# GenjiB/AVSiam

Measured on AMD Instinct MI355X. Metric: AV pretrain samples/sec (ViT-B/16, 75% mask), higher is better.
Workload: dtype bf16; 1 GPU; AVSiam pretrain step (contrastive + MAE passes, 2x Adam), ViT-B/16, 10 frames x196 + 512 audio tokens, 75% mask, batch 64/GPU; global_batch=64, frames=10, parallelism=dp1, residual_gradient_stream=bf16

## Files before the change

### avsiam_amd/csrc/gemm.hip

```cpp
#include "common.h"
#include <stdlib.h>
#include <type_traits>
#include <algorithm>
#include <numeric>

#define GLOBAL_AS __attribute__((address_space(1)))
#define LDS_AS __attribute__((address_space(3)))

constexpr int BM = 128, BN = 128, BK = 64;

struct GemmNtArgs {
    const bf16_t* A; long long lda;
    const bf16_t* B; long long ldb;
    int M, N, K;
    const float* bias;
    const float* res; long long ldr; const int* res_idx;
    const bf16_t* aux; long long ldaux;
    void* out; long long ldo; int out_f32;
    bf16_t* out2; long long ldo2;
    float alpha; int act;
    int scale_cols; float col_scale;
    float* colsum;
    int m_full;
    int m_split; const bf16_t* B2; const float* bias2; float* colsum2;
    uint8_t* out8; long long ldo8; float out8_scale;
    const float* qa; const float* qw; const float* qw2; float* q8;
    float q8_seen;
    int tb;
    int aux8;
};
#define GP8_BIAS 0.1296875f
#define GP8_STEPS 202.0f


typedef __attribute__((ext_vector_type(4))) uint32_t u32x4;

#ifndef NT8_ABLATE
#define NT8_ABLATE 0
#endif
#if NT8_ABLATE == 1
#define NT_STORE(ptr, val) asm volatile("" ::"v"(val))
#else
#define NT_STORE(ptr, val) *(ptr) = (val)
#endif

__device__ __forceinline__ void epi_apply4(float alpha, int ACT, float (&v)[4], const float4& bias4, uint2 p,
                                           bool has_res, f32x4 r) {
    v[0] += bias4.x; v[1] += bias4.y; v[2] += bias4.z; v[3] += bias4.w;
    if (ACT == 2) {
        v[0] *= __uint_as_float(p.x << 16);
        v[1] *= __uint_as_float(p.x & 0xffff0000u);
        v[2] *= __uint_as_float(p.y << 16);
        v[3] *= __uint_as_float(p.y & 0xffff0000u);
    }
    if (has_res) { v[0] += r[0]; v[1] += r[1]; v[2] += r[2]; v[3] += r[3]; }
    v[0] *= alpha; v[1] *= alpha; v[2] *= alpha; v[3] *= alpha;
}

template <int OFF>
__device__ __forceinline__ void epi_lds_w128(unsigned addr, const f32x4& v) {
    asm volatile("ds_write_b128 %0, %1 offset:%2" ::"v"(addr), "v"(v), "n"(OFF) : "memory");
}
template <int OFF>
__device__ __forceinline__ void epi_lds_r128(f32x4& v, unsigned addr) {
    asm volatile("ds_read_b128 %0, %1 offset:%2" : "=&v"(v) : "v"(addr), "n"(OFF) : "memory");
}
__device__ __forceinline__ void epi_lds_wait() {
    asm volatile("s_waitcnt lgkmcnt(0)" ::: "memory");
    __builtin_amdgcn_sched_barrier(0);
}

template <int MI>
struct EpiPrefetch {
    static constexpr int RG = 1;
    static constexpr int AG = MI < 4 ? MI : 4;
    static constexpr int NB = 3;
    f32x4 rs[NB][RG][4];
    u32x4 ax[AG][2];
};

template <int MI>
__device__ __forceinline__ void epi_load_res(const GemmNtArgs& a, f32x4 (&rs)[EpiPrefetch<MI>::RG][4], int grp, int lane, int mw0, int nw0) {
    const int n = nw0 + (lane & 15) * 4, rq = lane >> 4;
    if (a.res_idx) {
        int rrow[EpiPrefetch<MI>::RG][4];
#pragma unroll
        for (int mj = 0; mj < EpiPrefetch<MI>::RG; ++mj)
#pragma unroll
            for (int i = 0; i < 4; ++i) rrow[mj][i] = a.res_idx[min(mw0 + (grp * EpiPrefetch<MI>::RG + mj) * 16 + i * 4 + rq, a.M - 1)];
#pragma unroll
        for (int mj = 0; mj < EpiPrefetch<MI>::RG; ++mj)
#pragma unroll
            for (int i = 0; i < 4; ++i) rs[mj][i] = *reinterpret_cast<const f32x4*>(a.res + (long long)rrow[mj][i] * a.ldr + n);
    } else {
#pragma unroll
        for (int mj = 0; mj < EpiPrefetch<MI>::RG; ++mj)
#pragma unroll
            for (int i = 0; i < 4; ++i) {
                const int m = min(mw0 + (grp * EpiPrefetch<MI>::RG + mj) * 16 + i * 4 + rq, a.M - 1);
                rs[mj][i] = *reinterpret_cast<const f32x4*>(a.res + (long long)m * a.ldr + n);
            }
    }
}

template <int MI>
__device__ __forceinline__ void epi_load_aux(const GemmNtArgs& a, u32x4 (&ax)[EpiPrefetch<MI>::AG][2], int grp, int lane, int mw0, int nw0) {
    const int n = nw0 + (lane & 7) * 8, rq = lane >> 3;
#pragma unroll
    for (int mj = 0; mj < EpiPrefetch<MI>::AG; ++mj)
#pragma unroll
        for (int i = 0; i < 2; ++i) {
            const int m = min(mw0 + (grp * EpiPrefetch<MI>::AG + mj) * 16 + i * 8 + rq, a.M - 1);
            if (a.aux8) {
                const uint2 c = *reinterpret_cast<const uint2*>(reinterpret_cast<const uint8_t*>(a.aux) + (size_t)m * a.ldaux + n);
                ax[mj][i] = u32x4{c.x, c.y, 0u, 0u};
            } else
            ax[mj][i] = *reinterpret_cast<const u32x4*>(a.aux + (size_t)m * a.ldaux + n);
        }
}

template <int ACT, int MI>
__device__ __forceinline__ void nt_epilogue_prefetch(const GemmNtArgs& a, EpiPrefetch<MI>& pf, int lane, int mw0, int nw0) {
    if (ACT == 0 && a.out_f32 && a.res) {
#pragma unroll
        for (int g = 0; g < EpiPrefetch<MI>::NB - 1 && g < MI / EpiPrefetch<MI>::RG; ++g) epi_load_res<MI>(a, pf.rs[g], g, lane, mw0, nw0);
    }
}

__device__ __forceinline__ void nt_epilogue_stage_bias(const GemmNtArgs& a, char* smem, int wave, int lane, int mw0, int nw0) {
    float* sbias = reinterpret_cast<float*>(smem) + (blockDim.x >> 6) * (16 * 68) + wave * 64;
    const float* bias = mw0 >= a.m_split ? a.bias2 : a.bias;
    sbias[lane] = bias ? bias[nw0 + lane] : 0.f;
}

template <int ACT, int MI, int Q8 = 0>
__device__ __forceinline__ void nt_epilogue(const GemmNtArgs& a, f32x4 (&acc)[4][MI], EpiPrefetch<MI>& pf, char* smem, int wave, int lane,
                                            int mw0, int nw0, const int nrow = MI * 16) {
    const int fr = lane & 15, fq = lane >> 4;
    const unsigned smem_lds = (unsigned)(size_t)(LDS_AS const char*)smem;
    const unsigned stg_lds = smem_lds + wave * (16 * 68) * 4;
    const unsigned sbias_lds = smem_lds + ((blockDim.x >> 6) * (16 * 68) + wave * 64) * 4;
    const unsigned waddr = stg_lds + (fr * 68 + fq * 4) * 4;
    const float alpha = nw0 < a.scale_cols ? a.alpha * a.col_scale : a.alpha;
    float* const colsum = mw0 >= a.m_split ? a.colsum2 : a.colsum;
    if (ACT == 0 && a.out_f32) {
        const int cc = (lane & 15) * 4, rq = lane >> 4;
        const int n = nw0 + cc;
        float* stg = reinterpret_cast<float*>(smem) + wave * (16 * 68);
        const float* sbias = reinterpret_cast<const float*>(smem) + (blockDim.x >> 6) * (16 * 68) + wave * 64;
        constexpr int RG = EpiPrefetch<MI>::RG, NG = MI / RG, NB = EpiPrefetch<MI>::NB;
#pragma unroll
        for (int g = 0; g < NG; ++g) {
            if (g * RG * 16 >= nrow) continue;
            if (a.res && g + NB - 1 < NG) epi_load_res<MI>(a, pf.rs[(g + NB - 1) % NB], g + NB - 1, lane, mw0, nw0);
#pragma unroll
            for (int mj = 0; mj < RG; ++mj) {
                const int mi = g * RG + mj;
#pragma unroll
                for (int ni = 0; ni < 4; ++ni) *reinterpret_cast<f32x4*>(stg + fr * 68 + ni * 16 + fq * 4) = acc[ni][mi];
#pragma unroll
                for (int i = 0; i < 4; ++i) {
                    const int rr = i * 4 + rq;
                    const float4 t = *reinterpret_cast<const float4*>(stg + rr * 68 + cc);
                    const int m = mw0 + mi * 16 + rr;
                    if (m >= a.M) continue;
                    float v[4] = {t.x, t.y, t.z, t.w};
                    const float4 bias4 = *reinterpret_cast<const float4*>(sbias + cc);
                    epi_apply4(alpha, 0, v, bias4, make_uint2(0, 0), a.res != nullptr, pf.rs[g % NB][mj][i]);
                    NT_STORE(reinterpret_cast<f32x4*>(reinterpret_cast<float*>(a.out) + (size_t)m * a.ldo + n), (f32x4{v[0], v[1], v[2], v[3]}));
                }
            }
        }
    } else {
        const int cc = (lane & 7) * 8, rq = lane >> 3;
        const int n = nw0 + cc;
        const unsigned raddr = stg_lds + (rq * 68 + cc) * 4, baddr = sbias_lds + cc * 4;
        constexpr int AG = EpiPrefetch<MI>::AG, NG = MI / AG;
        float cs[8] = {0.f, 0.f, 0.f, 0.f, 0.f, 0.f, 0.f, 0.f};
        const float q8s = (Q8 != 0 && a.out8) ? a.out8_scale : 0.f;
        const float q8seen = a.q8_seen;
        float q8max = 0.f;
#pragma unroll
        for (int g = 0; g < NG; ++g) {
            if (g * AG * 16 >= nrow) continue;
            if (ACT == 2) epi_load_aux<MI>(a, pf.ax, g, lane, mw0, nw0);
#pragma unroll
            for (int mj = 0; mj < AG; ++mj) {
                const int mi = g * AG + mj;
                if (mi * 16 >= nrow) continue;
                epi_lds_w128<0>(waddr, acc[0][mi]); epi_lds_w128<64>(waddr, acc[1][mi]);
                epi_lds_w128<128>(waddr, acc[2][mi]); epi_lds_w128<192>(waddr, acc[3][mi]);
                f32x4 tq[2][2], bq[2];
                epi_lds_r128<0>(tq[0][0], raddr); epi_lds_r128<16>(tq[0][1], raddr);
                epi_lds_r128<2176>(tq[1][0], raddr); epi_lds_r128<2176 + 16>(tq[1][1], raddr);
                epi_lds_r128<0>(bq[0], baddr); epi_lds_r128<16>(bq[1], baddr);
                epi_lds_wait();
#pragma unroll
                for (int i = 0; i < 2; ++i) {
                    const int rr = i * 8 + rq;
                    const int m = mw0 + mi * 16 + rr;
                    if (m >= a.M) continue;
                    float v0[4] = {tq[i][0][0], tq[i][0][1], tq[i][0][2], tq[i][0][3]}, v1[4] = {tq[i][1][0], tq[i][1][1], tq[i][1][2], tq[i][1][3]};
                    u32x4 ax = {0, 0, 0, 0};
                    if (ACT == 2) ax = pf.ax[mj][i];
                    const f32x4 r0 = {0.f, 0.f, 0.f, 0.f}, r1 = r0;
                    const float4 bias_lo = make_float4(bq[0][0], bq[0][1], bq[0][2], bq[0][3]), bias_hi = make_float4(bq[1][0], bq[1][1], bq[1][2], bq[1][3]);
                    if (ACT == 2 && Q8 != 1 && a.aux8) {
                        auto dec = [](float b) { return fmaf(b, 1.0f / GP8_STEPS, -GP8_BIAS); };
                        const float g0[4] = {dec((float)((ax[0] >> 0) & 0xffu)), dec((float)((ax[0] >> 8) & 0xffu)),
                                             dec((float)((ax[0] >> 16) & 0xffu)), dec((float)((ax[0] >> 24) & 0xffu))};
                        const float g1[4] = {dec((float)((ax[1] >> 0) & 0xffu)), dec((float)((ax[1] >> 8) & 0xffu)),
                                             dec((float)((ax[1] >> 16) & 0xffu)), dec((float)((ax[1] >> 24) & 0xffu))};
                        epi_apply4(alpha, 0, v0, bias_lo, make_uint2(0, 0), false, r0);
                        epi_apply4(alpha, 0, v1, bias_hi, make_uint2(0, 0), false, r1);
#pragma unroll
                        for (int j = 0; j < 4; ++j) { v0[j] *= g0[j]; v1[j] *= g1[j]; }
                    } else {
                    epi_apply4(alpha, ACT, v0, bias_lo, make_uint2(ax[0], ax[1]), false, r0);
                    epi_apply4(alpha, ACT, v1, bias_hi, make_uint2(ax[2], ax[3]), false, r1);
                    }
                    if (colsum) {
#pragma unroll
                        for (int j = 0; j < 4; ++j) { cs[j] += v0[j]; cs[4 + j] += v1[j]; }
                    }
                    uint4 o;
                    if (ACT == 1) {
                        o.x = pack_bf2(gelu_erf_grad(v0[0]), gelu_erf_grad(v0[1])); o.y = pack_bf2(gelu_erf_grad(v0[2]), gelu_erf_grad(v0[3]));
                        o.z = pack_bf2(gelu_erf_grad(v1[0]), gelu_erf_grad(v1[1])); o.w = pack_bf2(gelu_erf_grad(v1[2]), gelu_erf_grad(v1[3]));
                    } else {
                        o.x = pack_bf2(v0[0], v0[1]); o.y = pack_bf2(v0[2], v0[3]);
                        o.z = pack_bf2(v1[0], v1[1]); o.w = pack_bf2(v1[2], v1[3]);
                    }
                    if (ACT == 1 && Q8 != 2 && a.aux8) {
                        auto enc = [](float g, unsigned sel, unsigned old) { return __builtin_amdgcn_cvt_pk_u8_f32(fmaf(g, GP8_STEPS, GP8_BIAS * GP8_STEPS), sel, old); };
                        unsigned c0 = enc(gelu_erf_grad(v0[0]), 0, 0); c0 = enc(gelu_erf_grad(v0[1]), 1, c0); c0 = enc(gelu_erf_grad(v0[2]), 2, c0); c0 = enc(gelu_erf_grad(v0[3]), 3, c0);
                        unsigned c1 = enc(gelu_erf_grad(v1[0]), 0, 0); c1 = enc(gelu_erf_grad(v1[1]), 1, c1); c1 = enc(gelu_erf_grad(v1[2]), 2, c1); c1 = enc(gelu_erf_grad(v1[3]), 3, c1);
                        *reinterpret_cast<uint2*>(reinterpret_cast<uint8_t*>(a.out) + (size_t)m * a.ldo + n) = make_uint2(c0, c1);
                    } else
                    if (Q8 != 2 || a.out) NT_STORE(reinterpret_cast<u32x4*>(reinterpret_cast<bf16_t*>(a.out) + (size_t)m * a.ldo + n), (u32x4{o.x, o.y, o.z, o.w}));
                    if (Q8 == 2 && ACT != 1 && a.out8) {
                        auto c8 = [&](float x) { q8max = fmaxf(q8max, fabsf(x)); return __builtin_amdgcn_fmed3f(x * q8s, -57344.f, 57344.f); };
                        int w0 = __builtin_amdgcn_cvt_pk_bf8_f32(c8(v0[0]), c8(v0[1]), 0, false);
                        w0 = __builtin_amdgcn_cvt_pk_bf8_f32(c8(v0[2]), c8(v0[3]), w0, true);
                        int w1 = __builtin_amdgcn_cvt_pk_bf8_f32(c8(v1[0]), c8(v1[1]), 0, false);
                        w1 = __builtin_amdgcn_cvt_pk_bf8_f32(c8(v1[2]), c8(v1[3]), w1, true);
                        *reinterpret_cast<uint2*>(a.out8 + (size_t)m * a.ldo8 + n) = make_uint2((unsigned)w0, (unsigned)w1);
                    }
                    if (ACT == 1) {
                        uint4 gq;
                        gq.x = pack_bf2(gelu_erf(v0[0]), gelu_erf(v0[1])); gq.y = pack_bf2(gelu_erf(v0[2]), gelu_erf(v0[3]));
                        gq.z = pack_bf2(gelu_erf(v1[0]), gelu_erf(v1[1])); gq.w = pack_bf2(gelu_erf(v1[2]), gelu_erf(v1[3]));
                        if (Q8 != 1 || a.out2) NT_STORE(reinterpret_cast<u32x4*>(a.out2 + (size_t)m * a.ldo2 + n), (u32x4{gq.x, gq.y, gq.z, gq.w}));
                        if (Q8 == 1 && a.out8) {
                            const float q = q8s;
                            auto q8 = [&](float x) { const float gx = gelu_erf(x); q8max = fmaxf(q8max, fabsf(gx)); return __builtin_amdgcn_fmed3f(gx * q, -448.f, 448.f); };
                            int w0 = __builtin_amdgcn_cvt_pk_fp8_f32(q8(v0[0]), q8(v0[1]), 0, false);
                            w0 = __builtin_amdgcn_cvt_pk_fp8_f32(q8(v0[2]), q8(v0[3]), w0, true);
                            int w1 = __builtin_amdgcn_cvt_pk_fp8_f32(q8(v1[0]), q8(v1[1]), 0, false);
                            w1 = __builtin_amdgcn_cvt_pk_fp8_f32(q8(v1[2]), q8(v1[3]), w1, true);
                            *reinterpret_cast<uint2*>(a.out8 + (size_t)m * a.ldo8 + n) = make_uint2((unsigned)w0, (unsigned)w1);
                        }
                    }
                }
            }
        }
        if (Q8 != 0 && a.out8 && a.q8) q_amax_update(a.q8, q8max, q8seen);
        if (colsum) {
#pragma unroll
            for (int j = 0; j < 8; ++j) {
                float t = cs[j];
                t += __shfl_xor(t, 8, 64);
                t += __shfl_xor(t, 16, 64);
                t += __shfl_xor(t, 32, 64);
                cs[j] = t;
            }
            if (rq == 0) {
#pragma unroll
                for (int j = 0; j < 8; ++j) atomicAdd(colsum + n + j, cs[j]);
            }
        }
    }
}

template <int ACT, int NWN, int MI>
__global__ __launch_bounds__(128 * NWN) void gemm_nt_kernel(GemmNtArgs a) {
    constexpr int NT = 128 * NWN;
    constexpr int TBM = 2 * MI * 16;
    constexpr int TBN = NWN * 64;
    constexpr int A_BYTES = TBM * 128, B_BYTES = TBN * 128, BUF_BYTES = A_BYTES + B_BYTES;
    constexpr int CA = TBM * 8 / NT, CB = TBN * 8 / NT;
// ... 21 lines not shown
            const int wg = xcd_remap(v, nfull);
            m0 = (wg / nt_n) * TBM;
            n0 = (wg % nt_n) * TBN;
        } else {
            const int h = v - nfull;
            m0 = a.m_full + (h / nt_n) * (TBM / 2);
            n0 = (h % nt_n) * TBN;
        }
#pragma unroll
        for (int i = 0; i < CA; ++i) {
            const int p = i * NT + tid, row = p >> 3, c = (p & 7) ^ (row & 7);
            srcA[i] = a.A + (size_t)min(m0 + row, a.M - 1) * a.lda + c * 8;
        }
#pragma unroll
        for (int i = 0; i < CB; ++i) {
            const int p = i * NT + tid, row = p >> 3, c = (p & 7) ^ (row & 7);
            srcB[i] = (m0 >= a.m_split ? a.B2 : a.B) + (size_t)(n0 + row) * a.ldb + c * 8;
        }
    };
    auto stage = [&](int buf, int k0) {
        char* sa = smem + buf * BUF_BYTES;
        char* sb = sa + A_BYTES;
#pragma unroll
        for (int i = 0; i < CA; ++i)
            if (i < CAH || !half)
                __builtin_amdgcn_global_load_lds((const GLOBAL_AS void*)(srcA[i] + k0), (LDS_AS void*)(sa + (i * NT + wave * 64) * 16), 16, 0, 0);
#pragma unroll
        for (int i = 0; i < CB; ++i)
            __builtin_amdgcn_global_load_lds((const GLOBAL_AS void*)(srcB[i] + k0), (LDS_AS void*)(sb + (i * NT + wave * 64) * 16), 16, 0, 0);
    };

    int v = blockIdx.x;
    if (v >= ntiles) return;
    set_tile(v);
    stage(0, 0);
    auto run_tile = [&](auto mit) {
        constexpr int MIT = decltype(mit)::value;
        f32x4 acc[4][MIT];
#pragma unroll
        for (int i = 0; i < 4; ++i)
#pragma unroll
            for (int j = 0; j < MIT; ++j) acc[i][j] = f32x4{0.f, 0.f, 0.f, 0.f};
        for (int t = 0; t < nk; ++t) {
            asm volatile("s_waitcnt vmcnt(0)" ::: "memory");
            __syncthreads();
            if (t + 1 < nk) stage((t + 1) & 1, (t + 1) * BK);
            const char* sa = smem + (t & 1) * BUF_BYTES + wm * (MIT * 16) * 128;
            const char* sb = smem + (t & 1) * BUF_BYTES + A_BYTES + wn * 64 * 128;
#pragma unroll
            for (int kk = 0; kk < 2; ++kk) {
                const int off = kk ? off_k1 : off_k0;
                bf16x8 wf[4], xf[MIT];
#pragma unroll
                for (int i = 0; i < 4; ++i) wf[i] = *reinterpret_cast<const bf16x8*>(sb + i * 16 * 128 + off);
#pragma unroll
                for (int i = 0; i < MIT; ++i) xf[i] = *reinterpret_cast<const bf16x8*>(sa + i * 16 * 128 + off);
                __builtin_amdgcn_s_setprio(1);
#pragma unroll
                for (int mi = 0; mi < MIT; ++mi)
#pragma unroll
                    for (int ni = 0; ni < 4; ++ni)
                        acc[ni][mi] = __builtin_amdgcn_mfma_f32_16x16x32_bf16(wf[ni], xf[mi], acc[ni][mi], 0, 0, 0);
                __builtin_amdgcn_s_setprio(0);
            }
        }
        const int em = m0 + wm * (MIT * 16), en = n0 + wn * 64;
        __syncthreads();
        nt_epilogue_stage_bias(a, smem + BUF_BYTES, wave, lane, em, en);
        const bool has_next = v + (int)gridDim.x < ntiles;
        EpiPrefetch<MIT> pf;
        nt_epilogue_prefetch<ACT, MIT>(a, pf, lane, em, en);
        nt_epilogue<ACT, MIT>(a, acc, pf, smem + BUF_BYTES, wave, lane, em, en);
        if (has_next) {
            set_tile(v + gridDim.x);
            stage(0, 0);
        }
    };
    for (; v < ntiles; v += gridDim.x) {
        if (!half) run_tile(std::integral_constant<int, MI>{});
        else run_tile(std::integral_constant<int, MIH>{});
    }
}

template <int N>
__device__ __forceinline__ void wait_vm() {
    asm volatile("" ::: "memory");
    __builtin_amdgcn_s_waitcnt((N & 15) | (7 << 4) | (15 << 8) | ((N >> 4) << 14));
    asm volatile("" ::: "memory");
}

template <int ACT, int FP8 = 0, int NBA = 4, int NBB = 4>
__global__ __launch_bounds__(512) void gemm_nt8_kernel(GemmNtArgs a) {
    constexpr int NT = 512, TBN = 256, MI = 8;
    constexpr int HA = 128 + 32 * NBA, HB = 128 + 32 * NBB;
    constexpr int A_BYTES = 256 * 128, BUF_BYTES = 2 * A_BYTES, GR = 16384;
    extern __shared__ __attribute__((aligned(16))) char smem[];
    const int tid = threadIdx.x, lane = tid & 63;
    const int wave = __builtin_amdgcn_readfirstlane(tid >> 6);
    const int g = wave >> 2, wc = wave & 3;
    const int nt_n = a.N / TBN;
    const int tb = NBA == NBB ? 0 : a.tb;
    const int rows_a = (tb / nt_n) * HA;
    const int ntiles = tb + ((a.M - rows_a + HB - 1) / HB) * nt_n;
    const int fr = lane & 15, fq = lane >> 4;
    const int off_k0 = fr * 128 + (((FP8 ? 2 * fq : 0 + fq) ^ (lane & 7)) << 4);
    const int off_k1 = fr * 128 + (((FP8 ? 2 * fq + 1 : 4 + fq) ^ (lane & 7)) << 4);
    const int nk = a.K / BK;
    const unsigned lds_base = (unsigned)(size_t)(LDS_AS const char*)smem;
    float dq_a = a.alpha, dq_b = a.alpha, q8_scale = a.out8_scale, q8_seen = 0.f;
    if (FP8) {
        if (a.qa) {
            const float ia = a.qa[AVS_Q_INV];
            dq_a = ia * a.qw[AVS_Q_INV];
            dq_b = ia * a.qw2[AVS_Q_INV];
        }
        if (a.out8 && a.q8) { q8_scale = a.q8[AVS_Q_SCALE]; q8_seen = a.q8[AVS_Q_AMAX]; }
        dq_a = __builtin_bit_cast(float, __builtin_amdgcn_readfirstlane(__builtin_bit_cast(int, dq_a)));
        dq_b = __builtin_bit_cast(float, __builtin_amdgcn_readfirstlane(__builtin_bit_cast(int, dq_b)));
        q8_scale = __builtin_bit_cast(float, __builtin_amdgcn_readfirstlane(__builtin_bit_cast(int, q8_scale)));
        q8_seen = __builtin_bit_cast(float, __builtin_amdgcn_readfirstlane(__builtin_bit_cast(int, q8_seen)));
    }

    const bf16_t* sA[2][2];
    const bf16_t* sB[2][2];
    int m0 = 0, n0 = 0;
    auto set_tile = [&](int v) {
#if NT8_ABLATE == 3
        const int wg = 0 * v;
#else
        const bool first = v < tb;
        const int wg = first ? xcd_remap(v, tb) : xcd_remap(v - tb, ntiles - tb);
#endif
        const int hg = first ? HA / 2 : HB / 2;
        m0 = first ? (wg / nt_n) * HA : rows_a + (wg / nt_n) * HB;
        n0 = (wg % nt_n) * TBN;
#pragma unroll
        for (int h = 0; h < 2; ++h)
#pragma unroll
            for (int j = 0; j < 2; ++j) {
                const int p = j * NT + tid, lr = p >> 3, c = (p & 7) ^ (lr & 7);
                sA[h][j] = a.A + (size_t)min(m0 + h * hg + lr, a.M - 1) * a.lda + c * 8;
                sB[h][j] = (m0 >= a.m_split ? a.B2 : a.B) + (size_t)(n0 + (lr >> 5) * 64 + h * 32 + (lr & 31)) * a.ldb + c * 8;
            }
    };
    auto dma_a = [&](int t, int h) {
        char* dst = smem + (t & 1) * BUF_BYTES + h * GR;
#pragma unroll
        for (int j = 0; j < 2; ++j)
            __builtin_amdgcn_global_load_lds((const GLOBAL_AS void*)(sA[h][j] + t * BK), (LDS_AS void*)(dst + (j * NT + wave * 64) * 16), 16, 0, 0);
    };
    auto dma_b = [&](int t, int h) {
        char* dst = smem + (t & 1) * BUF_BYTES + A_BYTES;
#pragma unroll
        for (int j = 0; j < 2; ++j) {
            const int lr0 = j * 64 + wave * 8;
            __builtin_amdgcn_global_load_lds((const GLOBAL_AS void*)(sB[h][j] + t * BK),
                                             (LDS_AS void*)(dst + ((lr0 >> 5) * 64 + h * 32 + (lr0 & 31)) * 128), 16, 0, 0);
        }
    };
    auto bar = [&]() {
        asm volatile("" ::: "memory");
        __builtin_amdgcn_s_barrier();
        asm volatile("" ::: "memory");
    };

    int v = blockIdx.x;
    if (v >= ntiles) return;
    set_tile(v);
    dma_a(0, 0); dma_a(0, 1); dma_b(0, 0); dma_b(0, 1);
    auto run_tile = [&](auto nbc) {
        constexpr int NB1 = decltype(nbc)::value, HG = 64 + 16 * NB1;
        f32x4 acc[4][MI];
#pragma unroll
        for (int i = 0; i < 4; ++i)
#pragma unroll
            for (int j = 0; j < MI; ++j) acc[i][j] = f32x4{0.f, 0.f, 0.f, 0.f};
#if NT8_ABLATE == 4
        f32x16 acc16[2][2][2];
#pragma unroll
        for (int i = 0; i < 8; ++i)
#pragma unroll
            for (int r = 0; r < 16; ++r) acc16[i >> 2][(i >> 1) & 1][i & 1][r] = 0.f;
#endif
        wait_vm<0>();
        bar();
        if (nk > 1) { dma_b(1, 0); dma_a(1, 0); }
        if (g == 1) bar();
        bf16x8 xf[4][2], wb[2][2][2];
        for (int t = 0; t < nk; ++t) {
            const unsigned la = lds_base + (t & 1) * BUF_BYTES + (g * 128) * 128;
            const unsigned lb = lds_base + (t & 1) * BUF_BYTES + A_BYTES + (wc * 64) * 128;
            const unsigned va0 = la + off_k0, va1 = la + off_k1, vb0 = lb + off_k0, vb1 = lb + off_k1;
            const bool n1 = t + 1 < nk, n2 = t + 2 < nk;
#define NT8_RD(dst, addr, OFF) asm volatile("ds_read_b128 %0, %1 offset:%2" : "=&v"(dst) : "v"(addr), "i"(OFF) : "memory")
#define NT8_RD_A(AH)                                                                                          \
    NT8_RD(xf[0][0], va0, (AH) * 8192 + 0);    NT8_RD(xf[0][1], va1, (AH) * 8192 + 0);                          \
    NT8_RD(xf[1][0], va0, (AH) * 8192 + 2048); NT8_RD(xf[1][1], va1, (AH) * 8192 + 2048);                       \
    NT8_RD(xf[2][0], va0, (AH) * 8192 + 4096); NT8_RD(xf[2][1], va1, (AH) * 8192 + 4096);                       \
    NT8_RD(xf[3][0], va0, (AH) * 8192 + 6144); NT8_RD(xf[3][1], va1, (AH) * 8192 + 6144)
#define NT8_RD_B(BH)                                                                                          \
    NT8_RD(wb[BH][0][0], vb0, (BH) * 4096 + 0);    NT8_RD(wb[BH][0][1], vb1, (BH) * 4096 + 0);                  \
    NT8_RD(wb[BH][1][0], vb0, (BH) * 4096 + 2048); NT8_RD(wb[BH][1][1], vb1, (BH) * 4096 + 2048)
            auto mma = [&](int ah, int bh) {
                asm volatile("s_waitcnt lgkmcnt(0)" ::: "memory");
                __builtin_amdgcn_sched_barrier(0);
                __builtin_amdgcn_s_setprio(1);
#if NT8_ABLATE == 4
#pragma unroll
                for (int kq = 0; kq < 4; ++kq)
#pragma unroll
                    for (int mb = 0; mb < 2; ++mb)
                        acc16[bh][ah][mb] = __builtin_amdgcn_mfma_f32_32x32x16_bf16(wb[bh][kq >> 1][kq & 1], xf[mb * 2 + (kq >> 1)][kq & 1], acc16[bh][ah][mb], 0, 0, 0);
#else
                if (FP8) {
                    typedef __attribute__((ext_vector_type(8))) int i32x8;
                    typedef __attribute__((ext_vector_type(4))) int i32x4;
#pragma unroll
                    for (int mi = 0; mi < 4; ++mi)
#pragma unroll
                        for (int ni = 0; ni < 2; ++ni) {
                            const i32x4 w0 = __builtin_bit_cast(i32x4, wb[bh][ni][0]), w1 = __builtin_bit_cast(i32x4, wb[bh][ni][1]);
                            const i32x4 x0 = __builtin_bit_cast(i32x4, xf[mi][0]), x1 = __builtin_bit_cast(i32x4, xf[mi][1]);
                            const i32x8 wv = {w0[0], w0[1], w0[2], w0[3], w1[0], w1[1], w1[2], w1[3]};
                            const i32x8 xv = {x0[0], x0[1], x0[2], x0[3], x1[0], x1[1], x1[2], x1[3]};
                            acc[bh * 2 + ni][ah * 4 + mi] =
                                __builtin_amdgcn_mfma_scale_f32_16x16x128_f8f6f4(wv, xv, acc[bh * 2 + ni][ah * 4 + mi], 0, FP8 == 2 ? 1 : 0, 0, 0, 0, 0);
                        }
                } else {
#pragma unroll
                    for (int kk = 0; kk < 2; ++kk)
#pragma unroll
                        for (int mi = 0; mi < 4; ++mi)
#pragma unroll
                            for (int ni = 0; ni < 2; ++ni) {
                                if (ah == 1 && mi >= NB1) continue;
                                acc[bh * 2 + ni][ah * 4 + mi] =
                                    __builtin_amdgcn_mfma_f32_16x16x32_bf16(wb[bh][ni][kk], xf[mi][kk], acc[bh * 2 + ni][ah * 4 + mi], 0, 0, 0);
                            }
                }
#endif
                __builtin_amdgcn_s_setprio(0);
                __builtin_amdgcn_sched_barrier(0);
            };
            NT8_RD_B(0); NT8_RD_A(0);
            if (n1) { dma_a(t + 1, 1); wait_vm<6>(); } else wait_vm<0>();
            bar(); mma(0, 0); bar();
            NT8_RD_B(1);
            if (n1) dma_b(t + 1, 1);
            bar(); mma(0, 1); bar();
            if (NB1 == 4) { NT8_RD_A(1); }
            else {
                NT8_RD(xf[0][0], va0, 8192 + 0);    NT8_RD(xf[0][1], va1, 8192 + 0);
                NT8_RD(xf[1][0], va0, 8192 + 2048); NT8_RD(xf[1][1], va1, 8192 + 2048);
                if (NB1 > 2) { NT8_RD(xf[2][0], va0, 8192 + 4096); NT8_RD(xf[2][1], va1, 8192 + 4096); }
            }
            if (n2) dma_b(t + 2, 0);
            bar(); mma(1, 1); bar();
            if (n2) { dma_a(t + 2, 0); wait_vm<6>(); }
            else if (n1) wait_vm<2>();
            bar(); mma(1, 0); bar();
        }
#undef NT8_RD
#undef NT8_RD_A
#undef NT8_RD_B
        if (g == 0) bar();
        const int em = m0 + g * HG, en = n0 + wc * 64;
        __syncthreads();
        nt_epilogue_stage_bias(a, smem + BUF_BYTES, wave, lane, em, en);
        const bool has_next = v + (int)gridDim.x < ntiles;
        int elane = lane;
        asm volatile("" : "+v"(elane));
        EpiPrefetch<MI> pf;
        nt_epilogue_prefetch<ACT, MI>(a, pf, elane, em, en);
        const bool early = has_next && ACT != 2 && !a.out_f32;
        int vnext = v + (int)gridDim.x;
        if (early) {
            set_tile(vnext);
            dma_a(0, 0); dma_a(0, 1); dma_b(0, 0); dma_b(0, 1);
        }
#if NT8_ABLATE >= 2
#pragma unroll
        for (int i = 0; i < 4; ++i)
#pragma unroll
            for (int j = 0; j < MI; ++j) asm volatile("" ::"v"(acc[i][j]));
#if NT8_ABLATE == 4
#pragma unroll
        for (int i = 0; i < 8; ++i) asm volatile("" ::"v"(acc16[i >> 2][(i >> 1) & 1][i & 1]));
#endif
#else
        if (FP8) {
            const float dq = m0 >= a.m_split ? dq_b : dq_a;
#pragma unroll
            for (int i = 0; i < 4; ++i)
#pragma unroll
                for (int j = 0; j < MI; ++j) acc[i][j] *= dq;
            GemmNtArgs e = a;
            e.alpha = 1.0f;
            e.out8_scale = q8_scale;
            e.q8_seen = q8_seen;
            nt_epilogue<ACT, MI, FP8>(e, acc, pf, smem + BUF_BYTES, wave, elane, em, en, HG);
        } else {
            nt_epilogue<ACT, MI>(a, acc, pf, smem + BUF_BYTES, wave, elane, em, en, HG);
        }
#endif
        wait_vm<0>();
        if (has_next) {
            asm volatile("" : "+s"(vnext));
            set_tile(vnext);
            if (!early) { dma_a(0, 0); dma_a(0, 1); dma_b(0, 0); dma_b(0, 1); }
        }
    };
    for (; v < ntiles; v += gridDim.x) {
        if (NBA != NBB && v < tb) run_tile(std::integral_constant<int, NBA>{});
        else run_tile(std::integral_constant<int, NBB>{});
    }
}

template <int ACT, int MI = 4>
__global__ __launch_bounds__(256) void gemm_nt_ring_kernel(GemmNtArgs a) {
    constexpr int NT = 256, NWN = 2, NS = 4;
    constexpr int TBM = 2 * MI * 16, TBN = 128;
    constexpr int A_BYTES = TBM * 128, B_BYTES = TBN * 128, SLOT = A_BYTES + B_BYTES;
    constexpr int CA = TBM * 8 / NT, CB = TBN * 8 / NT;
    constexpr int DPT = CA + CB;
    extern __shared__ __attribute__((aligned(16))) char smem[];
    const int tid = threadIdx.x, lane = tid & 63;
    const int wave = __builtin_amdgcn_readfirstlane(tid >> 6);
    const int wm = wave / NWN, wn = wave % NWN;
    const int nt_n = a.N / TBN;
    const int ntiles = ((a.M + TBM - 1) / TBM) * nt_n;
    const int v = blockIdx.x;
    if (v >= ntiles) return;
    const int fr = lane & 15, fq = lane >> 4;
    const int off_k0 = fr * 128 + (((0 + fq) ^ (lane & 7)) << 4);
    const int off_k1 = fr * 128 + (((4 + fq) ^ (lane & 7)) << 4);
    const int nk = a.K / BK;
    const int wg = xcd_remap(v, ntiles);
    const int m0 = (wg / nt_n) * TBM, n0 = (wg % nt_n) * TBN;
    const bf16_t* srcA[CA];
    const bf16_t* srcB[CB];
#pragma unroll
    for (int i = 0; i < CA; ++i) {
        const int p = i * NT + tid, row = p >> 3, c = (p & 7) ^ (row & 7);
        srcA[i] = a.A + (size_t)min(m0 + row, a.M - 1) * a.lda + c * 8;
    }
#pragma unroll
    for (int i = 0; i < CB; ++i) {
        const int p = i * NT + tid, row = p >> 3, c = (p & 7) ^ (row & 7);
        srcB[i] = (m0 >= a.m_split ? a.B2 : a.B) + (size_t)(n0 + row) * a.ldb + c * 8;
    }
    auto stage = [&](int slot, int k0) {
        char* sa = smem + slot * SLOT;
        char* sb = sa + A_BYTES;
#pragma unroll
        for (int i = 0; i < CA; ++i)
            __builtin_amdgcn_global_load_lds((const GLOBAL_AS void*)(srcA[i] + k0), (LDS_AS void*)(sa + (i * NT + wave * 64) * 16), 16, 0, 0);
#pragma unroll
        for (int i = 0; i < CB; ++i)
            __builtin_amdgcn_global_load_lds((const GLOBAL_AS void*)(srcB[i] + k0), (LDS_AS void*)(sb + (i * NT + wave * 64) * 16), 16, 0, 0);
    };
#pragma unroll
    for (int t = 0; t < NS - 1; ++t)
        if (t < nk) stage(t, t * BK);

    f32x4 acc[4][MI];
#pragma unroll
    for (int i = 0; i < 4; ++i)
#pragma unroll
        for (int j = 0; j < MI; ++j) acc[i][j] = f32x4{0.f, 0.f, 0.f, 0.f};
    const unsigned lds_base = (unsigned)(size_t)(LDS_AS const char*)smem;
    const unsigned la = lds_base + wm * (MI * 16) * 128, lb = lds_base + A_BYTES + wn * 64 * 128;
    int slot = 0;
    for (int t = 0; t < nk; ++t) {
        const int ahead = min(NS - 2, nk - 1 - t);
        if (ahead == 2) wait_vm<2 * DPT>();
        else if (ahead == 1) wait_vm<DPT>();
        else wait_vm<0>();
        asm volatile("" ::: "memory");
        __builtin_amdgcn_s_barrier();
        asm volatile("" ::: "memory");
        if (t + NS - 1 < nk) stage(slot == 0 ? NS - 1 : slot - 1, (t + NS - 1) * BK);
        const unsigned va0 = la + slot * SLOT + off_k0, va1 = la + slot * SLOT + off_k1;
        const unsigned vb0 = lb + slot * SLOT + off_k0, vb1 = lb + slot * SLOT + off_k1;
// ... 284 lines not shown
#pragma unroll
            for (int r = 0; r < 16; ++r) {
                const int n1 = n1_0 + wr * (MI * 32) + i * 32 + (r & 3) + 8 * (r >> 2) + 4 * h;
                atomicAdd(a.C + (size_t)n1 * a.ldc + n2, acc[i][j][r]);
            }
        }
}

#define g_force_tile (avs_tuning().gemm_tile)
#define g_persistent (avs_tuning().gemm_persistent)
#define g_nt8 (avs_tuning().gemm_nt8)
#define g_force_h (avs_tuning().nt_tile_h)

extern "C" int avs_gemm_set_persistent(int on) { return avs_tuning_set("gemm_persistent", on ? 1 : 0); }

static long long g_nt_dispatches = 0;
extern "C" long long avs_gemm_nt_dispatches(void) { return g_nt_dispatches; }

extern "C" int avs_gemm_set_nt8(int on) { return avs_tuning_set("gemm_nt8", on ? 1 : 0); }
extern "C" int avs_gemm_set_tile_height(int h) { return avs_tuning_set("nt_tile_h", h); }
extern "C" int avs_gemm_set_tile(int tile) { return avs_tuning_set("gemm_tile", tile); }

enum { NT_TWOBUF = 0, NT_RING = 1, NT_RING_HALF = 2, NT_TWOBUF_HALF = 3, NT_PERSISTENT = 4 };
static bool nt_use_big(int M, int N) {
    const int force = g_force_tile;
    const int big_tiles = ceil_div(M, 256) * (N / 256);
    const int big_min = avs_tuning().nt_big_min > 0 ? avs_tuning().nt_big_min : avs_persistent_slots() / 2;
    return force == 256 ? (N % 256) == 0 : force == 128 ? false : ((N % 256) == 0 && big_tiles >= big_min);
}
static int nt_small_family(int M, int N, int K, bool whole) {
    const int nwg = ceil_div(M, BM) * (N / BN);
    if (avs_tuning().gemm_ring == 2 && 2 * nwg <= avs_persistent_slots() && whole) return K >= 256 ? NT_RING_HALF : NT_TWOBUF_HALF;
    if (avs_tuning().gemm_ring && nwg <= avs_persistent_slots() && K >= 256 && whole) return NT_RING;
    return NT_TWOBUF;
}

extern "C" int avs_gemm_nt_plan(int M, int N, int K, int* family, int* workgroups) {
    AVS_CHECK_ARG(M > 0 && N > 0 && K > 0 && (N % BN) == 0 && (K % BK) == 0 && family && workgroups, "gemm_nt_plan: bad arguments M=%d N=%d K=%d", M, N, K);
    if (nt_use_big(M, N)) {
        const int tiles = ceil_div(M, 256) * (N / 256), slots = avs_persistent_slots();
        *family = NT_PERSISTENT;
        *workgroups = tiles < slots ? tiles : slots;
        return 0;
    }
    const int fam = nt_small_family(M, N, K, true);
    *family = fam;
    *workgroups = ceil_div(M, (fam == NT_RING_HALF || fam == NT_TWOBUF_HALF) ? BM / 2 : BM) * (N / BN);
    return 0;
}

static int gemm_nt_launch(const bf16_t* A, long long lda, const bf16_t* B, long long ldb, int M, int N, int K,
                          const float* bias, const float* res, long long ldr, const int* res_idx, const bf16_t* aux,
                          long long ldaux, void* out, long long ldo, int out_f32, bf16_t* out2, long long ldo2,
                          float alpha, int act, int scale_cols, float col_scale, float* colsum,
                          int m_split, const bf16_t* B2, const float* bias2, float* colsum2, hipStream_t stream) {
    AVS_CHECK_ARG(M > 0 && N > 0 && K > 0 && (N % BN) == 0 && (K % BK) == 0, "gemm_nt: need N%%128==0, K%%64==0 (M=%d N=%d K=%d)", M, N, K);
    AVS_CHECK_ARG(A && B && out, "gemm_nt: null operand");
    int aux8 = 0;
    if (out_f32 == 2) {
        AVS_CHECK_ARG(act == 1 && (ldo % 8) == 0 && ldo >= N, "gemm_nt: out_f32 == 2 (8-bit gelu') goes with act 1");
        out_f32 = 0; aux8 = 1;
    }
    if (act == 3) {
        AVS_CHECK_ARG(aux && ldaux >= N, "gemm_nt: act 3 (act 2 with 8-bit gelu' codes) needs aux");
        act = 2; aux8 = 1;
    }
    AVS_CHECK_ARG((lda % 8) == 0 && (ldb % 8) == 0 && (ldo % (out_f32 ? 4 : 8)) == 0 && (!out2 || (ldo2 % 8) == 0) && (!aux || (ldaux % 8) == 0),
                  "gemm_nt: leading dimensions must keep 16-byte alignment");
    AVS_CHECK_ARG(act >= 0 && act <= 2 && (act != 1 || out2) && (act != 2 || aux), "gemm_nt: bad activation arguments");
    AVS_CHECK_ARG(!(out_f32 && act != 0), "gemm_nt: fp32 output is supported with act 0 only");
    AVS_CHECK_ARG(!(out_f32 && colsum), "gemm_nt: the fused column sum is implemented for bf16 output");
    AVS_CHECK_ARG(!res || out_f32, "gemm_nt: the residual add is implemented for fp32 output");
    AVS_CHECK_ARG(scale_cols >= 0 && scale_cols <= N && (scale_cols % 64) == 0, "gemm_nt: scale_cols must be a multiple of 64 within N");
    GemmNtArgs a{A, lda, B, ldb, M, N, K, bias, res, ldr, res_idx, aux, ldaux, out, ldo, out_f32, out2, ldo2, alpha, act, scale_cols, col_scale, colsum, M,
                 m_split, B2, bias2, colsum2, nullptr, 0, 1.0f, nullptr, nullptr, nullptr, nullptr, 0.f, 0, aux8};
    const int big_tiles = ceil_div(M, 256) * (N / 256);
    const bool big = nt_use_big(M, N);
    static bool attr_done = false;
    if (!attr_done) {
        hipError_t e = hipSuccess;
        const void* big_k[3] = {(const void*)gemm_nt_kernel<0, 4, 8>, (const void*)gemm_nt_kernel<1, 4, 8>, (const void*)gemm_nt_kernel<2, 4, 8>};
        const void* k8[6] = {(const void*)gemm_nt8_kernel<0>, (const void*)gemm_nt8_kernel<1>, (const void*)gemm_nt8_kernel<2>,
                             (const void*)gemm_nt8_kernel<0, 0, 4, 3>, (const void*)gemm_nt8_kernel<1, 0, 4, 3>, (const void*)gemm_nt8_kernel<2, 0, 4, 3>};
        for (int i = 0; i < 6 && e == hipSuccess; ++i) e = hipFuncSetAttribute(k8[i], hipFuncAttributeMaxDynamicSharedMemorySize, 131072);
        const void* small_k[3] = {(const void*)gemm_nt_kernel<0, 2, 4>, (const void*)gemm_nt_kernel<1, 2, 4>, (const void*)gemm_nt_kernel<2, 2, 4>};
        const void* ring_k[3] = {(const void*)gemm_nt_ring_kernel<0>, (const void*)gemm_nt_ring_kernel<1>, (const void*)gemm_nt_ring_kernel<2>};
        const void* ring_h[3] = {(const void*)gemm_nt_ring_kernel<0, 2>, (const void*)gemm_nt_ring_kernel<1, 2>, (const void*)gemm_nt_ring_kernel<2, 2>};
        for (int i = 0; i < 3 && e == hipSuccess; ++i) e = hipFuncSetAttribute(ring_h[i], hipFuncAttributeMaxDynamicSharedMemorySize, 98304);
        for (int i = 0; i < 3 && e == hipSuccess; ++i) {
            e = hipFuncSetAttribute(big_k[i], hipFuncAttributeMaxDynamicSharedMemorySize, 131072);
            if (e == hipSuccess) e = hipFuncSetAttribute(small_k[i], hipFuncAttributeMaxDynamicSharedMemorySize, 65536);
            if (e == hipSuccess) e = hipFuncSetAttribute(ring_k[i], hipFuncAttributeMaxDynamicSharedMemorySize, 131072);
        }
        if (e != hipSuccess) {
            avs_set_error("gemm_nt: hipFuncSetAttribute failed: %s", hipGetErrorString(e));
            return -1;
        }
        attr_done = true;
    }
    auto launch_small = [&](const GemmNtArgs& x) {
        const int nwg = ceil_div(x.M, BM) * (x.N / BN);
        const int fam = nt_small_family(x.M, x.N, x.K, x.m_full >= x.M);
        if (fam == NT_RING_HALF || fam == NT_TWOBUF_HALF) {
            const int nh = ceil_div(x.M, BM / 2) * (x.N / BN);
            if (fam == NT_RING_HALF) {
                if (act == 0) gemm_nt_ring_kernel<0, 2><<<nh, 256, 98304, stream>>>(x);
                else if (act == 1) gemm_nt_ring_kernel<1, 2><<<nh, 256, 98304, stream>>>(x);
                else gemm_nt_ring_kernel<2, 2><<<nh, 256, 98304, stream>>>(x);
                return;
            }
            GemmNtArgs h = x;
            h.m_full = 0;
            if (act == 0) gemm_nt_kernel<0, 2, 4><<<nh, 256, 65536, stream>>>(h);
            else if (act == 1) gemm_nt_kernel<1, 2, 4><<<nh, 256, 65536, stream>>>(h);
            else gemm_nt_kernel<2, 2, 4><<<nh, 256, 65536, stream>>>(h);
            return;
        }
        if (fam == NT_RING) {
            if (act == 0) gemm_nt_ring_kernel<0><<<nwg, 256, 131072, stream>>>(x);
            else if (act == 1) gemm_nt_ring_kernel<1><<<nwg, 256, 131072, stream>>>(x);
            else gemm_nt_ring_kernel<2><<<nwg, 256, 131072, stream>>>(x);
            return;
        }
        if (act == 0) gemm_nt_kernel<0, 2, 4><<<nwg, 256, 65536, stream>>>(x);
        else if (act == 1) gemm_nt_kernel<1, 2, 4><<<nwg, 256, 65536, stream>>>(x);
        else gemm_nt_kernel<2, 2, 4><<<nwg, 256, 65536, stream>>>(x);
    };
    if (big) {
        const int ncu = avs_persistent_slots();
        const int nt_n = N / 256, nt_m = ceil_div(M, 256);
        GemmNtArgs b = a;
        if (g_persistent && g_force_tile == 0 && big_tiles > ncu) {
            const int rows_full = ((big_tiles / ncu) * ncu) / nt_n;
            if (rows_full >= 1 && rows_full < nt_m && (big_tiles % ncu) * 2 <= ncu) b.m_full = rows_full * 256;
        }
        if (g_nt8 >= 1 && K >= 128 && g_persistent && g_force_tile == 0) {
            const bool one_set = m_split >= M || m_split <= 0;
            const int unit = nt_n * 8 / std::gcd(nt_n, 8);
            int tb = -1;
            if (one_set && g_force_h == 224) tb = 0;
            else if (one_set && g_force_h == 240) tb = ((nt_m / 2) * nt_n / unit) * unit;
            else if (g_force_h == 0) {
                const int rounds = ceil_div(nt_m * nt_n, ncu);
                const int nrt = (rounds * ncu) / nt_n;
                int b = (int)(((long long)nrt * 256 - M) / 32);
                if (b > nrt) b = nrt;
                if (b > 0) {
                    int ta = ((nrt - b) * nt_n + unit - 1) / unit * unit;
                    if (!one_set && ta / nt_n * 256 < m_split) ta = ceil_div(ceil_div(m_split, 256) * nt_n, unit) * unit;
                    if (ta / nt_n <= nrt) {
                        const int na = ta / nt_n, nb = ceil_div(M - (na * 256 < M ? na * 256 : M), 224);
                        const int nbig = ceil_div(ta, ncu), nall = ceil_div((na + nb) * nt_n, ncu);
                        const double cost = nbig + 0.90 * (nall - nbig);
                        if (nb > 0 && nall <= rounds && cost < 0.98 * rounds) tb = ta;
                    }
                }
            }
            a.tb = tb < 0 ? 0 : tb;
            const int tiles8 = tb < 0 ? nt_m * nt_n : tb + ceil_div(M - (tb / nt_n) * 256 > 0 ? M - (tb / nt_n) * 256 : 0, 224) * nt_n;
            int grid8 = tiles8 < ncu ? tiles8 : ncu;
            { const int gcap = avs_tuning().nt_grid; if (gcap > 0 && gcap < grid8) grid8 = gcap; }
#define NT8_LAUNCH(ACT_)                                                                          \
    do {                                                                                          \
        if (tb >= 0) gemm_nt8_kernel<ACT_, 0, 4, 3><<<grid8, 512, 131072, stream>>>(a);           \
        else gemm_nt8_kernel<ACT_, 0, 4, 4><<<grid8, 512, 131072, stream>>>(a);                   \
    } while (0)
            if (act == 0) NT8_LAUNCH(0);
            else if (act == 1) NT8_LAUNCH(1);
            else NT8_LAUNCH(2);
#undef NT8_LAUNCH
            AVS_LAUNCH_CHECK("gemm_nt8");
            ++g_nt_dispatches;
            return 0;
        }
        const int tiles_b = ceil_div(b.m_full, 256) * nt_n + (b.m_full < M ? ceil_div(M - b.m_full, 128) * nt_n : 0);
        const int grid = g_persistent ? (tiles_b < ncu ? tiles_b : ncu) : tiles_b;
        if (act == 0) gemm_nt_kernel<0, 4, 8><<<grid, 512, 131072, stream>>>(b);
        else if (act == 1) gemm_nt_kernel<1, 4, 8><<<grid, 512, 131072, stream>>>(b);
        else gemm_nt_kernel<2, 4, 8><<<grid, 512, 131072, stream>>>(b);
    } else {
        launch_small(a);
    }
    AVS_LAUNCH_CHECK("gemm_nt");
    ++g_nt_dispatches;
    return 0;
}

extern "C" int avs_gemm_nt_bf16(const bf16_t* A, long long lda, const bf16_t* B, long long ldb, int M, int N, int K,
                                const float* bias, const float* res, long long ldr, const int* res_idx, const bf16_t* aux,
                                long long ldaux, void* out, long long ldo, int out_f32, bf16_t* out2, long long ldo2,
                                float alpha, int act, int scale_cols, float col_scale, float* colsum, hipStream_t stream) {
    return gemm_nt_launch(A, lda, B, ldb, M, N, K, bias, res, ldr, res_idx, aux, ldaux, out, ldo, out_f32, out2, ldo2, alpha, act, scale_cols,
                          col_scale, colsum, 0x7fffffff, nullptr, nullptr, nullptr, stream);
}

extern "C" int avs_gemm_nt_fp8(const uint8_t* A, long long lda, const uint8_t* B, long long ldb, int M, int N, int K, const float* bias,
                               const float* res, long long ldr, void* out, long long ldo, int out_f32, bf16_t* out2, long long ldo2, float alpha,
                               int act, int scale_cols, float col_scale, uint8_t* out8, long long ldo8, float out8_scale,
                               const float* qa, const float* qw, float* q8, int m_split, const uint8_t* B2, const float* bias2, const float* qw2,
                               int a_e5m2, const bf16_t* aux, long long ldaux, float* colsum, float* colsum2, hipStream_t stream) {
    const bool gp8 = (out_f32 == 2) || (a_e5m2 == 2);
    AVS_CHECK_ARG(out_f32 != 2 || (act == 1 && !a_e5m2 && out && (ldo % 8) == 0 && ldo >= N), "gemm_nt_fp8: out_f32 == 2 (8-bit gelu') goes with act 1 of the forward form");
    AVS_CHECK_ARG(a_e5m2 != 2 || (act == 2 && aux && ldaux >= N), "gemm_nt_fp8: a_e5m2 == 2 (8-bit gelu' operand) goes with act 2");
    if (out_f32 == 2) out_f32 = 0;
    if (a_e5m2 == 2) a_e5m2 = 1;
    AVS_CHECK_ARG(!out8 || ((ldo8 % 8) == 0 && ldo8 >= N && (a_e5m2 ? act != 1 : act == 1)),
                  "gemm_nt_fp8: out8 = e4m3(gelu(x)) goes with act 1, out8 = e5m2(out) with the input-gradient form");
    AVS_CHECK_ARG(M > 0 && N > 0 && K >= 256 && (N % 256) == 0 && (K % 128) == 0, "gemm_nt_fp8: need N%%256==0, K%%128==0, K>=256 (M=%d N=%d K=%d)", M, N, K);
    AVS_CHECK_ARG(A && B && (out || (out8 && a_e5m2 && !out_f32)) && (lda % 16) == 0 && (ldb % 16) == 0 && lda >= K && ldb >= K && (!out || (ldo % (out_f32 ? 4 : 8)) == 0),
                  "gemm_nt_fp8: operands must keep 16-byte alignment (out may be NULL only beside an e5m2 out8)");
    AVS_CHECK_ARG(!res || out_f32, "gemm_nt_fp8: the residual add is implemented for fp32 output");
    AVS_CHECK_ARG((act == 0 && !out2) || (act == 1 && (out2 || out8) && !out_f32 && (!out2 || (ldo2 % 8) == 0) && !a_e5m2) ||
                  (act == 2 && a_e5m2 && aux && !out2 && !out_f32 && (ldaux % 8) == 0),
                  "gemm_nt_fp8: act 0; act 1 with a bf16 output pair (forward; out2 may be NULL beside out8); act 2 with aux (input-gradient form)");
    AVS_CHECK_ARG(!colsum || (!out_f32 && a_e5m2), "gemm_nt_fp8: the fused column sum goes with the bf16 output of the input-gradient form");
    AVS_CHECK_ARG(scale_cols >= 0 && scale_cols <= N && (scale_cols % 64) == 0, "gemm_nt_fp8: scale_cols must be a multiple of 64 within N");
    AVS_CHECK_ARG((qa == nullptr) == (qw == nullptr), "gemm_nt_fp8: qa and qw go together");
    const bool dual = m_split > 0 && m_split < M;
    AVS_CHECK_ARG(!dual || ((m_split % 256) == 0 && B2 && (bias == nullptr) == (bias2 == nullptr) && qa && qw2 && (colsum == nullptr) == (colsum2 == nullptr)),
                  "gemm_nt_fp8: two weight sets need m_split %% 256 == 0, B2, bias2 / colsum2 mirroring bias / colsum, and device records (qa, qw, qw2)");
    static bool attr_done = false;
    if (!attr_done) {
        const void* ks[4] = {(const void*)gemm_nt8_kernel<0, 1>, (const void*)gemm_nt8_kernel<1, 1>, (const void*)gemm_nt8_kernel<0, 2>, (const void*)gemm_nt8_kernel<2, 2>};
        for (int i = 0; i < 4; ++i)
            if (hipFuncSetAttribute(ks[i], hipFuncAttributeMaxDynamicSharedMemorySize, 131072) != hipSuccess) {
                avs_set_error("gemm_nt_fp8: hipFuncSetAttribute failed");
                return -1;
            }
        attr_done = true;
    }
    GemmNtArgs a{reinterpret_cast<const bf16_t*>(A), lda / 2, reinterpret_cast<const bf16_t*>(B), ldb / 2, M, N, K / 2, bias, res, ldr, nullptr, aux, ldaux,
                 out, ldo, out_f32, out2, ldo2, alpha, act, scale_cols, col_scale, colsum, M, dual ? m_split : 0x7fffffff,
                 dual ? reinterpret_cast<const bf16_t*>(B2) : nullptr, dual ? bias2 : nullptr, dual ? colsum2 : nullptr,
                 out8, ldo8, out8_scale, qa, qw, dual ? qw2 : qw, q8, 0.f};
    a.aux8 = gp8 ? 1 : 0;
    const int ncu = avs_persistent_slots();
    const int tiles = ceil_div(M, 256) * (N / 256);
    const int grid = tiles < ncu ? tiles : ncu;
    if (a_e5m2) {
        if (act == 0) gemm_nt8_kernel<0, 2><<<grid, 512, 131072, stream>>>(a);
        else gemm_nt8_kernel<2, 2><<<grid, 512, 131072, stream>>>(a);
    } else {
        if (act == 0) gemm_nt8_kernel<0, 1><<<grid, 512, 131072, stream>>>(a);
        else gemm_nt8_kernel<1, 1><<<grid, 512, 131072, stream>>>(a);
    }
    AVS_LAUNCH_CHECK("gemm_nt_fp8");
    return 0;
}
// ... 297 lines not shown
```

Before: 397.8 samples/s.

## Stream GELU-derivative byte codes into LDS via async DMA during GEMM mainloop

```diff
diff --git a/avsiam_amd/csrc/gemm.hip b/avsiam_amd/csrc/gemm.hip
--- a/avsiam_amd/csrc/gemm.hip
+++ b/avsiam_amd/csrc/gemm.hip
@@ -28,6 +28,7 @@
     float q8_seen;
     int tb;
     int aux8;
+    int aux_dma;
 };
 #define GP8_BIAS 0.1296875f
 #define GP8_STEPS 202.0f
@@ -133,9 +134,33 @@
     sbias[lane] = bias ? bias[nw0 + lane] : 0.f;
 }
 
-template <int ACT, int MI, int Q8 = 0>
+template <int N>
+__device__ __forceinline__ void wait_vm() {
+    asm volatile("" ::: "memory");
+    __builtin_amdgcn_s_waitcnt((N & 15) | (7 << 4) | (15 << 8) | ((N >> 4) << 14));
+    asm volatile("" ::: "memory");
+}
+
+typedef __attribute__((ext_vector_type(2))) uint32_t u32x2;
+template <int OFF>
+__device__ __forceinline__ void epi_lds_r64(u32x2& v, unsigned addr) {
+    asm volatile("ds_read_b64 %0, %1 offset:%2" : "=&v"(v) : "v"(addr), "n"(OFF) : "memory");
+}
+constexpr int NT8_CODE_LDS = 32768, NT8_CODE_SLOT = 1024;
+__device__ __forceinline__ void epi_dma_codes(const GemmNtArgs& a, char* cslot, int lane, int mw0, int nw0, int b0, int nblk) {
+    const uint8_t* src = reinterpret_cast<const uint8_t*>(a.aux) + nw0 + (lane & 3) * 16;
+#pragma unroll
+    for (int b = 0; b < 4; ++b) {
+        if (b0 + b >= nblk) continue;
+        const int m = min(mw0 + (b0 + b) * 16 + (lane >> 2), a.M - 1);
+        __builtin_amdgcn_global_load_lds((const GLOBAL_AS void*)(src + (size_t)m * a.ldaux), (LDS_AS void*)(cslot + b * NT8_CODE_SLOT), 16, 0, 0);
+    }
+}
+
+template <int ACT, int MI, int Q8 = 0, int DMA = 0>
 __device__ __forceinline__ void nt_epilogue(const GemmNtArgs& a, f32x4 (&acc)[4][MI], EpiPrefetch<MI>& pf, char* smem, int wave, int lane,
-                                            int mw0, int nw0, const int nrow = MI * 16) {
+                                            int mw0, int nw0, const int nrow = MI * 16, char* cslot = nullptr) {
+    static_assert(!DMA || (ACT == 2 && MI == 8 && Q8 == 0), "LDS-DMA delivery of the GELU' codes: gemm_nt8_kernel's bf16 ACT 2 epilogue");
     const int fr = lane & 15, fq = lane >> 4;
     const unsigned smem_lds = (unsigned)(size_t)(LDS_AS const char*)smem;
     const unsigned stg_lds = smem_lds + wave * (16 * 68) * 4;
@@ -180,10 +205,31 @@
         const float q8s = (Q8 != 0 && a.out8) ? a.out8_scale : 0.f;
         const float q8seen = a.q8_seen;
         float q8max = 0.f;
+        u32x2 cx[AG][2];
+        const unsigned caddr = (unsigned)(size_t)(LDS_AS const char*)cslot + lane * 8;
 #pragma unroll
         for (int g = 0; g < NG; ++g) {
             if (g * AG * 16 >= nrow) continue;
-            if (ACT == 2) epi_load_aux<MI>(a, pf.ax, g, lane, mw0, nw0);
+            if (ACT == 2 && DMA) {
+                if (g == 1) {
+                    if (NT8_ABLATE == 0 && mw0 + AG * 16 <= a.M) wait_vm<2 * AG>();
+                    else wait_vm<0>();
+                }
+#pragma unroll
+                for (int mj = 0; mj < AG; ++mj) {
+                    if ((g * AG + mj) * 16 >= nrow) continue;
+                    if (mj == 0) { epi_lds_r64<0>(cx[0][0], caddr); epi_lds_r64<512>(cx[0][1], caddr); }
+                    if (mj == 1) { epi_lds_r64<1024>(cx[1][0], caddr); epi_lds_r64<1024 + 512>(cx[1][1], caddr); }
+                    if (mj == 2) { epi_lds_r64<2048>(cx[2][0], caddr); epi_lds_r64<2048 + 512>(cx[2][1], caddr); }
+                    if (mj == 3) { epi_lds_r64<3072>(cx[3][0], caddr); epi_lds_r64<3072 + 512>(cx[3][1], caddr); }
+                }
+                epi_lds_wait();
+                if (g == 0) {
+                    epi_dma_codes(a, cslot, lane, mw0, nw0, AG, nrow / 16);
+                    asm volatile("" ::: "memory");
+                    __builtin_amdgcn_sched_barrier(0);
+                }
+            } else if (ACT == 2) epi_load_aux<MI>(a, pf.ax, g, lane, mw0, nw0);
 #pragma unroll
             for (int mj = 0; mj < AG; ++mj) {
                 const int mi = g * AG + mj;
@@ -202,10 +248,11 @@
                     if (m >= a.M) continue;
                     float v0[4] = {tq[i][0][0], tq[i][0][1], tq[i][0][2], tq[i][0][3]}, v1[4] = {tq[i][1][0], tq[i][1][1], tq[i][1][2], tq[i][1][3]};
                     u32x4 ax = {0, 0, 0, 0};
-                    if (ACT == 2) ax = pf.ax[mj][i];
+                    if (ACT == 2 && DMA) ax = u32x4{cx[mj][i][0], cx[mj][i][1], 0u, 0u};
+                    else if (ACT == 2) ax = pf.ax[mj][i];
                     const f32x4 r0 = {0.f, 0.f, 0.f, 0.f}, r1 = r0;
                     const float4 bias_lo = make_float4(bq[0][0], bq[0][1], bq[0][2], bq[0][3]), bias_hi = make_float4(bq[1][0], bq[1][1], bq[1][2], bq[1][3]);
-                    if (ACT == 2 && Q8 != 1 && a.aux8) {
+                    if (ACT == 2 && Q8 != 1 && (DMA || a.aux8)) {
                         auto dec = [](float b) { return fmaf(b, 1.0f / GP8_STEPS, -GP8_BIAS); };
                         const float g0[4] = {dec((float)((ax[0] >> 0) & 0xffu)), dec((float)((ax[0] >> 8) & 0xffu)),
                                              dec((float)((ax[0] >> 16) & 0xffu)), dec((float)((ax[0] >> 24) & 0xffu))};
@@ -393,13 +440,6 @@
     }
 }
 
-template <int N>
-__device__ __forceinline__ void wait_vm() {
-    asm volatile("" ::: "memory");
-    __builtin_amdgcn_s_waitcnt((N & 15) | (7 << 4) | (15 << 8) | ((N >> 4) << 14));
-    asm volatile("" ::: "memory");
-}
-
 template <int ACT, int FP8 = 0, int NBA = 4, int NBB = 4>
 __global__ __launch_bounds__(512) void gemm_nt8_kernel(GemmNtArgs a) {
     constexpr int NT = 512, TBN = 256, MI = 8;
@@ -495,6 +535,13 @@
 #endif
         wait_vm<0>();
         bar();
+        const bool cdma = ACT == 2 && FP8 == 0 && a.aux_dma;
+        char* const cslot = smem + 2 * BUF_BYTES + wave * (4 * NT8_CODE_SLOT);
+        if (cdma) {
+            int hlane = lane;
+            asm volatile("" : "+v"(hlane));
+            epi_dma_codes(a, cslot, hlane, m0 + g * HG, n0 + wc * 64, 0, HG / 16);
+        }
         if (nk > 1) { dma_b(1, 0); dma_a(1, 0); }
         if (g == 1) bar();
         bf16x8 xf[4][2], wb[2][2][2];
@@ -583,7 +630,7 @@
         asm volatile("" : "+v"(elane));
         EpiPrefetch<MI> pf;
         nt_epilogue_prefetch<ACT, MI>(a, pf, elane, em, en);
-        const bool early = has_next && ACT != 2 && !a.out_f32;
+        const bool early = has_next && (ACT != 2 || cdma) && !a.out_f32;
         int vnext = v + (int)gridDim.x;
         if (early) {
             set_tile(vnext);
@@ -610,6 +657,8 @@
             e.out8_scale = q8_scale;
             e.q8_seen = q8_seen;
             nt_epilogue<ACT, MI, FP8>(e, acc, pf, smem + BUF_BYTES, wave, elane, em, en, HG);
+        } else if (ACT == 2 && cdma) {
+            nt_epilogue<ACT, MI, 0, ACT == 2>(a, acc, pf, smem + BUF_BYTES, wave, elane, em, en, HG, cslot);
         } else {
             nt_epilogue<ACT, MI>(a, acc, pf, smem + BUF_BYTES, wave, elane, em, en, HG);
         }
@@ -1060,7 +1109,8 @@
         const void* big_k[3] = {(const void*)gemm_nt_kernel<0, 4, 8>, (const void*)gemm_nt_kernel<1, 4, 8>, (const void*)gemm_nt_kernel<2, 4, 8>};
         const void* k8[6] = {(const void*)gemm_nt8_kernel<0>, (const void*)gemm_nt8_kernel<1>, (const void*)gemm_nt8_kernel<2>,
                              (const void*)gemm_nt8_kernel<0, 0, 4, 3>, (const void*)gemm_nt8_kernel<1, 0, 4, 3>, (const void*)gemm_nt8_kernel<2, 0, 4, 3>};
-        for (int i = 0; i < 6 && e == hipSuccess; ++i) e = hipFuncSetAttribute(k8[i], hipFuncAttributeMaxDynamicSharedMemorySize, 131072);
+        for (int i = 0; i < 6 && e == hipSuccess; ++i)
+            e = hipFuncSetAttribute(k8[i], hipFuncAttributeMaxDynamicSharedMemorySize, 131072 + (i % 3 == 2 ? NT8_CODE_LDS : 0));
         const void* small_k[3] = {(const void*)gemm_nt_kernel<0, 2, 4>, (const void*)gemm_nt_kernel<1, 2, 4>, (const void*)gemm_nt_kernel<2, 2, 4>};
         const void* ring_k[3] = {(const void*)gemm_nt_ring_kernel<0>, (const void*)gemm_nt_ring_kernel<1>, (const void*)gemm_nt_ring_kernel<2>};
         const void* ring_h[3] = {(const void*)gemm_nt_ring_kernel<0, 2>, (const void*)gemm_nt_ring_kernel<1, 2>, (const void*)gemm_nt_ring_kernel<2, 2>};
@@ -1135,13 +1185,15 @@
                 }
             }
             a.tb = tb < 0 ? 0 : tb;
+            a.aux_dma = act == 2 && aux8 && (reinterpret_cast<uintptr_t>(aux) % 16) == 0 && (ldaux % 16) == 0;
+            const int lds8 = 131072 + (a.aux_dma ? NT8_CODE_LDS : 0);
             const int tiles8 = tb < 0 ? nt_m * nt_n : tb + ceil_div(M - (tb / nt_n) * 256 > 0 ? M - (tb / nt_n) * 256 : 0, 224) * nt_n;
             int grid8 = tiles8 < ncu ? tiles8 : ncu;
             { const int gcap = avs_tuning().nt_grid; if (gcap > 0 && gcap < grid8) grid8 = gcap; }
 #define NT8_LAUNCH(ACT_)                                                                          \
     do {                                                                                          \
-        if (tb >= 0) gemm_nt8_kernel<ACT_, 0, 4, 3><<<grid8, 512, 131072, stream>>>(a);           \
-        else gemm_nt8_kernel<ACT_, 0, 4, 4><<<grid8, 512, 131072, stream>>>(a);                   \
+        if (tb >= 0) gemm_nt8_kernel<ACT_, 0, 4, 3><<<grid8, 512, lds8, stream>>>(a);             \
+        else gemm_nt8_kernel<ACT_, 0, 4, 4><<<grid8, 512, lds8, stream>>>(a);                     \
     } while (0)
             if (act == 0) NT8_LAUNCH(0);
             else if (act == 1) NT8_LAUNCH(1);
```

Result: no change. 398.6 samples/s (median of 6 runs) (+0.2%).
